# OthmanB/TAMCMC-C

Measured on AMD Instinct MI355X. Metric: MCMC samples/sec (whole node), 1e5 nu-bins x 100 params x 20 tempered chains, higher is better.
Workload: dtype f64

## Files before the change

### tamcmc-c_amd/csrc/dev_step_impl.h

```cpp

struct FusedArgs {
    int NS;
    int xsplit;
    double *cand_vars, *cand_params;
    double *cand_logPr;
    int *cand_rej;
    int *cand_stP, *cand_stR;
    tamcmc_multiplet *mults;
    int *pairs, *nh, *nn;
    double *noise;
    double *bg;
    int *slot;
    double *prop_logPr;
    int *prop_st;
    double *quick;
    double *part;
    double *psum;
    double *lz;
    double qmargin;
    unsigned long long *qcount;
};

constexpr int QN = 8;
constexpr int ST_L = 1, ST_BR = 2, ST_ENTRY = 4, ST_LZ = 8, ST_FIRST = 16, ST_COMMIT = 32;
// ... 117 lines not shown
        if (stm == TAMCMC_OK && !(lp == -INFINITY || isnan(lp))) {
            const double cur = settled ? a.logPost_cur[q * C + m] : d.o.logPost;
            Sstar = -((log(u) - lp + cur) * Tm) / (double)a.pl;
            if (isfinite(Sstar)) ok = 1;
        } else if (u > 0.0) ok = 2;
        w[0] = Sstar; w[1] = ok; w[2] = -(double)a.pl / Tm; w[3] = settled ? a.logL_cur[q * C + m] : d.o.logL;
        double lus = 0, k1 = 0, k2 = 0;
        if (is_swap_iter(a, it)) {
            double us;
            if (swap_first(a, it, &us) == m) {
                const double TB = a.Tcoefs[m + 1];
                lus = log(us); k1 = Tm / TB - 1.0; k2 = TB / Tm - 1.0;
            }
        }
        w[4] = lus; w[5] = k1; w[6] = k2; w[7] = (double)slot;
    }
    if (settled) return;
    const double *sv, *sp;
    if (d.src_acc) {
        const size_t gp = (size_t)((it - 1) % 3) * f.NS + d.src_ps;
        sv = f.cand_vars + gp * Nv;
        sp = f.cand_params + gp * Np;
    } else {
        sv = a.vars_cur + ((size_t)d.src_par * C + d.src) * Nv;
        sp = a.params_cur + ((size_t)d.src_par * C + d.src) * Np;
    }
    double *dv = a.vars_cur + ((size_t)q * C + m) * Nv, *dp = a.params_cur + ((size_t)q * C + m) * Np;
    double *rv = (a.samples && rec >= 0) ? a.samples + ((size_t)rec * C + m) * Nv : nullptr;
    for (int i = lane; i < Nv; i += 64) { const double v = sv[i]; dv[i] = v; if (rv) rv[i] = v; }
    for (int i = lane; i < Np; i += 64) dp[i] = sp[i];
    if (lane == 0) {
        a.logL_cur[q * C + m] = d.o.logL;
        a.logPr_cur[q * C + m] = d.o.logPr;
        a.logPost_cur[q * C + m] = d.o.logPost;
        f.slot[q * C + m] = slot;
        a.moved[m] = d.src_acc;
        a.Pmove[m] = d.r;
        if (m == 0 && d.src_acc) a.counters[1] += 1;
        a.counters[8 + m] += d.src_acc;
        if (m == 0) a.counters[0] = it;
        if (d.swap_first == m) {
            atomicAdd((unsigned long long *)&a.counters[2], 1ull);
            if (d.swapped) atomicAdd((unsigned long long *)&a.counters[3], 1ull);
        }
        if (a.stats && rec >= 0) {
            double *r = a.stats + ((size_t)rec * C + m) * 3;
            r[0] = d.o.logL; r[1] = d.o.logPr; r[2] = d.o.logPost;
        }
        if (tiles && d.swap_first < 0 && f.quick[((size_t)(q ^ 1) * C + m) * QN + 1] == 2.0) atomicAdd(f.qcount + 1, 1ull);
    }
}


template <bool PAIR>
__device__ __forceinline__ void quick_sums(const double *c0, int n, int lane, double &s0, double &a0, double &s1, double &a1) {
    for (int t0 = 0; t0 < n; t0 += 256) {
        double v[4], w[4];
#pragma unroll
        for (int k = 0; k < 4; k++) {
            const int t = t0 + k * 64 + lane;
            v[k] = t < n ? c0[t] : 0.0;
            if (PAIR) w[k] = t < n ? c0[n + t] : 0.0;
        }
#pragma unroll
        for (int k = 0; k < 4; k++) {
            s0 += v[k]; a0 += fabs(v[k]);
            if (PAIR) { s1 += w[k]; a1 += fabs(w[k]); }
        }
    }
#pragma unroll
    for (int off = 32; off >= 1; off >>= 1) {
        s0 += __shfl_xor(s0, off, 64); a0 += __shfl_xor(a0, off, 64);
        if (PAIR) { s1 += __shfl_xor(s1, off, 64); a1 += __shfl_xor(a1, off, 64); }
    }
}
__device__ __forceinline__ int quick_decide_core(const DevSamplerArgs *ga, const FusedArgs *gf, int m, int q, int pairA, Decided *out) {
    const ConstArgs &a = *(const ConstArgs *)uniform_ptr(ga);
    const ConstFused &f = *(const ConstFused *)uniform_ptr(gf);
    const int lane = threadIdx.x & 63, C = a.C;
    const int p = q ^ 1, n = a.ntiles;
    const bool in_pair = pairA >= 0 && (m == pairA || m == pairA + 1);
    const int j0 = in_pair ? pairA : m;
    const double *c0 = f.psum + ((size_t)p * C + j0) * n;
    const double *r0 = f.quick + ((size_t)p * C + j0) * QN;
    double rec, s0 = 0, a0 = 0, s1 = 0, a1 = 0;
    if (in_pair) {
        rec = lane < 2 * QN ? r0[lane] : 0.0;
        quick_sums<true>(c0, n, lane, s0, a0, s1, a1);
    } else {
        rec = lane < QN ? r0[lane] : 0.0;
        quick_sums<false>(c0, n, lane, s0, a0, s1, a1);
    }
    const double St0 = __shfl(rec, 0, 64), ok0 = __shfl(rec, 1, 64);
    const int ps0 = (int)__shfl(rec, 7, 64);
    const double mg = f.qmargin;
    int acc0 = 0;
    if (ok0 == 2.0) { s0 = 0; a0 = 0; }
    else if (ok0 > 0 && fabs(s0 - St0) > mg * (a0 + fabs(St0))) acc0 = s0 < St0 ? 1 : 0;
    else return -1;
    Decided d;
    d.swap_first = -1; d.swapped = 0; d.src_par = p; d.r = 0;
    d.o.acc = 0; d.o.r = 0; d.o.logL = 0; d.o.logPr = 0; d.o.logPost = 0;
    if (!in_pair) { d.slot = 2 * m + acc0; d.src = m; d.src_acc = acc0; d.src_ps = ps0; }
    else {
        const double St1 = __shfl(rec, QN, 64), ok1 = __shfl(rec, QN + 1, 64);
        const int ps1 = (int)__shfl(rec, QN + 7, 64);
        int acc1 = 0;
        if (ok1 == 2.0) { s1 = 0; a1 = 0; }
        else if (ok1 > 0 && fabs(s1 - St1) > mg * (a1 + fabs(St1))) acc1 = s1 < St1 ? 1 : 0;
        else return -1;
        const double c0 = __shfl(rec, 2, 64), c1 = __shfl(rec, QN + 2, 64);
        const double LA = acc0 ? c0 * s0 : __shfl(rec, 3, 64), LB = acc1 ? c1 * s1 : __shfl(rec, QN + 3, 64);
        const double lus = __shfl(rec, 4, 64), x = LA * __shfl(rec, 5, 64) + LB * __shfl(rec, 6, 64);
        if (!(fabs(x - lus) > mg * (fabs(c0) * a0 + fabs(c1) * a1 + fabs(LA) + fabs(LB)))) return -1;
        const int swapped = x > lus ? 1 : 0;
        const int A = pairA, B = pairA + 1;
        d.swap_first = A; d.swapped = swapped;
        if (swapped) {
            if (m == A) { d.slot = 2 * C + (A >= f.xsplit ? 4 : 0) + acc1; d.src = B; d.src_acc = acc1; d.src_ps = ps1; }
            else { d.slot = 2 * C + (B >= f.xsplit ? 4 : 0) + 2 + acc0; d.src = A; d.src_acc = acc0; d.src_ps = ps0; }
        } else {
            if (m == A) { d.slot = 2 * A + acc0; d.src = A; d.src_acc = acc0; d.src_ps = ps0; }
            else { d.slot = 2 * B + acc1; d.src = B; d.src_acc = acc1; d.src_ps = ps1; }
        }
    }
    if (out && lane == 0) *out = d;
    return d.slot;
}
__device__ __attribute__((noinline)) int quick_decide_leaf(const DevSamplerArgs *ga, const FusedArgs *gf, int m, int q, int pairA, Decided *out) {
    return quick_decide_core(ga, gf, m, q, pairA, out);
}

__device__ __forceinline__ int quick_decide(const DevSamplerArgs *ga, const FusedArgs *gf, int m, long it, int q, int settled, int pairA,
                                            Decided *out) {
    if (settled) return decide(ga, gf, m, it, q, 1, out);
    const int s = quick_decide_leaf(ga, gf, m, q, pairA, out);
    return s >= 0 ? s : decide(ga, gf, m, it, q, 0, out);
}

__device__ __attribute__((noinline)) int decide_counted(const DevSamplerArgs *ga, const FusedArgs *gf, int m, long it, int q, int tile) {
    if (tile == 0 && (threadIdx.x & 63) == 0) atomicAdd(((const ConstFused *)uniform_ptr(gf))->qcount, 1ull);
    return decide(ga, gf, m, it, q, 0, nullptr);
}

struct StepTiles {
    const DevSamplerArgs *ga;
    const FusedArgs *gf;
    long it;
    int q, first, settled, pairA;
    static constexpr bool coherent_partials = false;
    static constexpr bool early_loads = true;
    __device__ __forceinline__ tile::SlotWords head(const LoglikeArgs &a, int b, int tile) const {
        const int m = first + b;
        if (settled) return tile::slot_words(a, decide(ga, gf, m, it, q, 1, nullptr));
        const bool lone = a.per > 0 && !(pairA >= 0 && (m == pairA || m == pairA + 1));
        tile::SlotWords w0{}, w1{};
        if (lone) { w0 = tile::slot_words(a, 2 * m); w1 = tile::slot_words(a, 2 * m + 1); }
        int s = quick_decide_core(ga, gf, m, q, pairA, nullptr);
        if (s < 0) s = decide_counted(ga, gf, m, it, q, tile);
        if (lone && (s >> 1) == m) return (s & 1) ? w1 : w0;
        return tile::slot_words(a, s);
    }
    __device__ __forceinline__ void store_sums(int b, int tile, double s0, double s1) const {
        const ConstArgs &a = *(const ConstArgs *)uniform_ptr(ga);
        const ConstFused &f = *(const ConstFused *)uniform_ptr(gf);
        f.psum[((size_t)q * a.C + first + b) * a.ntiles + tile] = s0 + s1;
    }
    __device__ __forceinline__ void operator()(int, int, int) const {}
};

__device__ __attribute__((noinline)) void role_prior(const DevSamplerArgs *ga, const FusedArgs *gf, size_t gs, int h, const double *s_vars,
                                                     const double *s_params, const UnpackLds *Up) {
    const DevSamplerArgs &a = *ga;
    const FusedArgs &f = *gf;
    const UnpackLds U = *Up;
    const int Nv = a.Nv, Np = a.desc.Np, tid = threadIdx.x;
    if (h == 0) {
        for (int i = tid; i < Nv; i += 64) f.cand_vars[gs * Nv + i] = s_vars[i];
        for (int i = tid; i < Np; i += 64) f.cand_params[gs * Np + i] = s_params[i];
    }
    int rej = 0;
#ifdef TAMCMC_PROBE
    long ps_[4] = {0, 0, 0, 0};
    const double fh = wave_log_prior_part(a.desc, s_params, U, TB - 128, h, &rej, ps_);
    if (tid == 0 && (int)(gs % f.NS) == 2) { long *w = a.counters + 8 + a.C + 16 * h + 4; w[0] += ps_[1] - ps_[0]; w[1] += ps_[2] - ps_[1]; }
#else
    const double fh = wave_log_prior_part(a.desc, s_params, U, TB - 128, h, &rej);
#endif
    if (tid == 0) {
        f.cand_logPr[2 * gs + h] = fh;
        f.cand_stP[2 * gs + h] = *U.status;
        if (h == 0) f.cand_rej[gs] = rej;
    }
}
__device__ __forceinline__ TablePtrs candidate_tables(const DevSamplerArgs &a, const FusedArgs &f, int q_dst) {
    TablePtrs T;
    T.mults = f.mults + (size_t)q_dst * f.NS * a.desc.per; T.pairs = f.pairs + (size_t)q_dst * 2 * f.NS; T.nh = f.nh + (size_t)q_dst * f.NS;
    T.nn = f.nn + (size_t)q_dst * f.NS; T.noise = f.noise + (size_t)q_dst * f.NS * a.desc.stride;
    T.bg = nullptr; T.ntiles = a.ntiles; T.tile_bins = a.tile_bins;
    return T;
}
__device__ __attribute__((noinline)) void role_rows(const DevSamplerArgs *ga, const FusedArgs *gf, int q_dst, int slot, size_t gs,
                                                    const double *s_params, const UnpackLds *Up) {
    const DevSamplerArgs &a = *ga;
    const FusedArgs &f = *gf;
    const UnpackLds U = *Up;
    if (threadIdx.x == 0) mt::shared_scalars_base(a.desc.model_id, s_params, a.desc.plength, *U.S);
    __syncthreads();
    const TablePtrs T = candidate_tables(a, f, q_dst);
#ifdef TAMCMC_PROBE
    __shared__ long ps_[8];
    wg_unpack(a.desc, s_params, U, slot, T, true, false, false, true, ps_);
    __syncthreads();
    if (threadIdx.x == 0 && (int)(gs % f.NS) == 2) {
        long *w = a.counters + 8 + a.C + 8 + 4; w[0] += ps_[1] - ps_[0]; w[1] += ps_[2] - ps_[1];
        long *v = a.counters + 8 + a.C + 32; v[0] += ps_[5] - ps_[4]; v[1] += ps_[6] - ps_[5]; v[2] += ps_[7] - ps_[6]; v[3] += 1;
    }
#else
    wg_unpack(a.desc, s_params, U, slot, T, true, false, false, true);
#endif
    if (threadIdx.x == 0) f.cand_stR[gs] = *U.status;
}
__device__ __attribute__((noinline)) void role_background(const DevSamplerArgs *ga, const FusedArgs *gf, int q_dst, int slot, int role,
                                                          const double *s_params, const UnpackLds *Up) {
    const DevSamplerArgs &a = *ga;
    const FusedArgs &f = *gf;
    const UnpackLds U = *Up;
    if (!f.bg) return;
    if (threadIdx.x == 0) mt::shared_scalars_base(a.desc.model_id, s_params, a.desc.plength, *U.S);
    __syncthreads();
    TablePtrs T = candidate_tables(a, f, q_dst);
    T.bg = f.bg + (size_t)q_dst * f.NS * a.ntiles * bg::NH;
    const int quarter = (a.ntiles + 3) / 4, k = role - 3;
    wg_bg_tiles(a.desc, s_params, U.S, slot, T, 0, 64, k * quarter, (k + 1) * quarter);
}

__device__ __attribute__((noinline)) void lz_normals(const DevSamplerArgs *ga, long itn, int m, double *s_z) {
    normals_into(*ga, m, itn, s_z);
}
__device__ __attribute__((noinline)) void lz_rows(const DevSamplerArgs *ga, const FusedArgs *gf, int q_dst, int m, const double *s_z) {
    Lz_rows_wave(*ga, m, s_z, gf->lz + ((size_t)q_dst * ga->C + m) * ga->Nv);
}
__device__ __forceinline__ void lz_block(const DevSamplerArgs *ga, const FusedArgs *gf, long itn, int q_dst, int m, unsigned char *lds) {
    double *s_z = (double *)lds;
    lz_normals(ga, itn, m, s_z);
    __syncthreads();
    lz_rows(ga, gf, q_dst, m, s_z);
}

__device__ void candidate_role(const DevSamplerArgs &a, const FusedArgs &f, const DevSamplerArgs *ga, const FusedArgs *gf, long itn, int q_src,
                               int q_dst, int slot, int role, bool entry, int settled, int pairA, unsigned char *lds, Decided *dec) {
    if (role > 6) return;
    const int C = a.C, Nv = a.Nv, Np = a.desc.Np, tid = threadIdx.x;
    const int e_dst = (int)(itn % 3);
    int m, src, on_prop;
    if (slot < 2 * C) { m = slot >> 1; src = m; on_prop = slot & 1; }
    else {
        if (entry || !is_swap_iter(a, itn - 1)) return;
        const int A = swap_first(a, itn - 1, nullptr), e = slot - 2 * C;
        m = (e < 2) ? A : A + 1;
        src = (e < 2) ? A + 1 : A;
        on_prop = e & 1;
        slot += (m >= f.xsplit) ? 4 : 0;
    }
    if (entry && on_prop) return;
    if (entry && role == 0 && tid == 0) f.slot[q_src * C + m] = 2 * m;
#ifdef TAMCMC_PROBE
    long pt[6];
    pt[0] = (long)wall_clock64();
#define RSTAMP(k) pt[k] = (long)wall_clock64()
#else
#define RSTAMP(k)
#endif
    double *s_params = (double *)lds;
    double *s_vars = s_params + Np;
    double *s_z = s_vars + Nv;
    const UnpackLds U = carve_unpack_lds((unsigned char *)(s_z + Nv + 1));
    __shared__ UnpackLds s_U;
    if (tid == 0) s_U = U;
    const double *bv, *bp;
    if (entry) {
        bv = a.vars_cur + ((size_t)q_src * C + src) * Nv;
        bp = a.params_cur + ((size_t)q_src * C + src) * Np;
    } else {
        const int ps = quick_decide(ga, gf, src, itn - 1, q_src, settled, pairA, dec);
        __syncthreads();
        const Decided d = *dec;
        if (on_prop) {
            const size_t gp = (size_t)((itn - 1) % 3) * f.NS + ps;
            bv = f.cand_vars + gp * Nv;
            bp = f.cand_params + gp * Np;
        } else if (d.src_acc) {
            const size_t gp = (size_t)((itn - 2) % 3) * f.NS + d.src_ps;
            bv = f.cand_vars + gp * Nv;
            bp = f.cand_params + gp * Np;
        } else {
            bv = a.vars_cur + ((size_t)d.src_par * C + d.src) * Nv;
            bp = a.params_cur + ((size_t)d.src_par * C + d.src) * Np;
        }
    }
    RSTAMP(1);
    const double *lz = f.lz + ((size_t)q_dst * C + m) * Nv;
    constexpr int PW = (int)(sizeof(mt::PolyTab) / sizeof(double));
    if (Nv <= 128 && Np <= 128 && PW <= 256) {
        double r_v[2], r_z[2], r_p[2], r_t[4];
        int r_i[2];
#pragma unroll
        for (int e = 0; e < 2; e++) {
            const int i = tid + 64 * e;
            r_v[e] = i < Nv ? bv[i] : 0.0; r_z[e] = i < Nv ? lz[i] : 0.0; r_i[e] = i < Nv ? a.index_to_relax[i] : 0;
            r_p[e] = i < Np ? bp[i] : 0.0;
        }
// ... 108 lines not shown
```

### tamcmc-c_amd/csrc/loglike_tile.h

```cpp
#pragma once
#include <hip/hip_runtime.h>
#include <stdint.h>

#include "kernels.h"
#include "bg_series.h"

namespace tamcmc {
namespace tile {

constexpr int CHUNK = 64;

constexpr int F_FULL = 1;
constexpr int F_SAFE = 2;
constexpr int F_ASYM = 4;
constexpr int F_FAR = 8;

constexpr int M_STRICT = 0, M_FAST_DIRECT = 2, M_FAST = 1;

constexpr int NC = 16;
constexpr double RHO_MAX2 = 1.0 / 36.0;
constexpr double RHO_MAX2_ASYM = 1.0 / 64.0;
constexpr int NH = bg::NH;
constexpr int ROW = NC + 2;

struct __attribute__((aligned(16))) LdsMult {
    int i0, i1, l, flags;
    double g;
    double asym;
    double c2sq;
    double fcx;
    double2 nh[7];
};

__device__ __forceinline__ double rcp_nr1(double d) {
    double r = __builtin_amdgcn_rcp(d);
    return fma(fma(-d, r, 1.0), r, r);
}
__device__ __forceinline__ double rcp_nr2(double d) {
    double r = __builtin_amdgcn_rcp(d);
    r = fma(fma(-d, r, 1.0), r, r);
    return fma(fma(-d, r, 1.0), r, r);
}

template <int NV, int WGS = 256>
__device__ __forceinline__ void block_reduce(double (&v)[NV], double *s_red, double *out) {
    const int lane = threadIdx.x & 63, wave = threadIdx.x >> 6;
#pragma unroll
    for (int i = 0; i < NV; i++) {
#pragma unroll
        for (int off = 32; off >= 1; off >>= 1) v[i] = v[i] + __shfl_down(v[i], off, 64);
    }
    if (lane == 0) {
#pragma unroll
        for (int i = 0; i < NV; i++) s_red[wave * NV + i] = v[i];
    }
    __syncthreads();
    if (threadIdx.x == 0) {
#pragma unroll
        for (int i = 0; i < NV; i++) {
            double s = s_red[i];
            for (int w = 1; w < WGS / 64; w++) s = s + s_red[w * NV + i];
            out[i] = s;
        }
    }
}

template <int NM, int K, bool FULL>
__device__ __forceinline__ void strict_mult(const LdsMult &M, const double (&xv)[K], const int (&bin)[K], double (&acc)[K]) {
    double nu[NM], hv[NM];
#pragma unroll
    for (int m = 0; m < NM; m++) {
        const double2 p = M.nh[m];
        nu[m] = p.x;
        hv[m] = p.y;
    }
    const double g2 = M.g;
    const int i0 = M.i0, i1 = M.i1;
    if (!(M.flags & F_ASYM)) {
#pragma unroll
        for (int k = 0; k < K; k++) {
            if (FULL || (bin[k] >= i0 && bin[k] < i1)) {
                double res = 0.0;
#pragma unroll
                for (int m = 0; m < NM; m++) {
                    const double d = xv[k] - nu[m];
                    double p = d * d;
                    p = 4.0 * p / g2;
                    const double inv = 1.0 / (1.0 + p);
                    res = res + hv[m] * inv;
                }
                acc[k] = acc[k] + res;
            }
        }
    } else {
        const double asym = M.asym, fc = M.fcx, c2sq = M.c2sq;
#pragma unroll
        for (int k = 0; k < K; k++) {
            if (FULL || (bin[k] >= i0 && bin[k] < i1)) {
                const double t = 1.0 + asym * (xv[k] / fc - 1.0);
                const double asy = t * t + c2sq;
                double res = 0.0;
#pragma unroll
                for (int m = 0; m < NM; m++) {
                    const double d = xv[k] - nu[m];
                    double p = d * d;
                    p = 4.0 * p / g2;
                    const double inv = 1.0 / (1.0 + p);
                    res = res + hv[m] * (asy * inv);
                }
                acc[k] = acc[k] + res;
            }
        }
    }
}

template <int NM, int K, bool FULL>
__device__ __forceinline__ void fast_mult(const LdsMult &M, const double (&xv)[K], const int (&bin)[K], double (&acc)[K], double xc) {
    double nA[NM], hv[NM];
#pragma unroll
    for (int m = 0; m < NM; m++) {
        const double2 p = M.nh[m];
        nA[m] = -p.x;
        hv[m] = p.y;
    }
    const double g = M.g;
    const int i0 = M.i0, i1 = M.i1;
    const int flags = M.flags;
    if (flags & F_SAFE) {
        const bool has_asym = flags & F_ASYM;
        const double afc = M.fcx, c2sq = M.c2sq, one_m_asym = 1.0 - M.asym;
#pragma unroll
        for (int k = 0; k < K; k++) {
            if (FULL || (bin[k] >= i0 && bin[k] < i1)) {
                const double xx = xv[k];
                const double dx = xx - xc;
                double t = fma(dx, g, nA[0]);
                double D = fma(t, t, 1.0);
                double N = hv[0];
#pragma unroll
                for (int m = 1; m < NM; m++) {
                    t = fma(dx, g, nA[m]);
                    const double q = fma(t, t, 1.0);
                    N = fma(N, q, hv[m] * D);
                    D = D * q;
                }
                double res = N * rcp_nr1(D);
                if (has_asym) {
                    const double ta = fma(afc, xx, one_m_asym);
                    res = res * fma(ta, ta, c2sq);
                }
                acc[k] = acc[k] + res;
            }
            if (K > 4 && (k & 3) == 3) __builtin_amdgcn_sched_barrier(0);
        }
    } else {
#pragma unroll
        for (int k = 0; k < K; k++) {
            if (FULL || (bin[k] >= i0 && bin[k] < i1)) {
                const double xx = xv[k];
                const double dx = xx - xc;
                double res = 0.0;
#pragma unroll
                for (int m = 0; m < NM; m++) {
                    const double t = fma(dx, g, nA[m]);
                    res = res + hv[m] / fma(t, t, 1.0);
                }
                if (flags & F_ASYM) {
                    const double ta = fma(M.fcx, xx, 1.0 - M.asym);
                    res = res * fma(ta, ta, M.c2sq);
                }
                acc[k] = acc[k] + res;
            }
        }
    }
}

template <bool FAST, int NM, int K>
__device__ __forceinline__ void mult_dispatch(const LdsMult &M, const double (&xv)[K], const int (&bin)[K], double (&acc)[K], double xc) {
    if (M.flags & F_FULL) {
        if (FAST) fast_mult<NM, K, true>(M, xv, bin, acc, xc);
        else strict_mult<NM, K, true>(M, xv, bin, acc);
    } else {
        if (FAST) fast_mult<NM, K, false>(M, xv, bin, acc, xc);
        else strict_mult<NM, K, false>(M, xv, bin, acc);
    }
}


template <int MODE, int WGS>
struct __attribute__((aligned(16))) TileLds {
    static constexpr bool FARFIELD = (MODE == M_FAST);
    static constexpr int LDS_BYTES = FARFIELD ? (WGS * ROW * 8 > CHUNK * (int)sizeof(LdsMult) ? WGS * ROW * 8 : CHUNK * (int)sizeof(LdsMult))
                                              : CHUNK * (int)sizeof(LdsMult);
    unsigned char buf[LDS_BYTES];
    double coef[NC];
    double part[WGS / 16][NC];
    double red[2 * (WGS / 64)];
    double lt[TAMCMC_MAX_HARVEY];
    double lto[TAMCMC_MAX_HARVEY];
    int n, nfar, anyfar;
    unsigned short slot[CHUNK * 7];
};

template <int MODE, int WGS, int K, bool WRITE_MODEL, bool DELTA, class Tail>
__device__ __forceinline__ void tile_compute(const LoglikeArgs &a, const int tile, const int b, const int sb, TileLds<MODE, WGS> &S, const int mbeg,
                                             const int mend, const int nh, const int nn, const Tail &tail, const double *xpre) {
    constexpr bool FAST = (MODE != M_STRICT);
    constexpr bool COH = Tail::coherent_partials;
    static_assert(!DELTA || (FAST && !WRITE_MODEL), "DELTA launches are FAST-mode, logL-only");
    constexpr bool FARFIELD = (MODE == M_FAST);
    LdsMult *s_m = (LdsMult *)S.buf;
    double *s_rows = (double *)S.buf;
    int &s_n = S.n, &s_nfar = S.nfar, &s_anyfar = S.anyfar;
    unsigned short *s_slot = S.slot;
    double *s_coef = S.coef;
    double(*s_part)[NC] = S.part;
    double *s_red = S.red;
    double *s_lt = S.lt, *s_lto = S.lto;
    const int tid = threadIdx.x;
#ifdef TAMCMC_PROBE
#define KSTAMP(k) do { if (a.dbg && b == 0 && tile == a.ntiles / 2 && tid == 0) a.dbg[k] = (long)wall_clock64(); } while (0)
#define PROBE_SKIP(bit) (a.probe & (bit))
    const long wg_t0 = (a.dbg && a.dbg[7] == 77) ? (long)wall_clock64() : 0;
#else
#define KSTAMP(k) do { } while (0)
#define PROBE_SKIP(bit) false
#endif
    KSTAMP(0);
    constexpr int TILE = WGS * K;
    const int t0 = tile * TILE;
    const int t1 = min(t0 + TILE, a.Nx);
    if (DELTA) {
        if (a.d_done && a.d_done[(size_t)b * a.ntiles + tile]) return;
        const int lo = a.d_range[2 * b], hi = a.d_range[2 * b + 1];
        if (t1 <= lo || t0 >= hi) {
            if (tid == 0) {
                double *p = a.partials + ((size_t)b * a.ntiles + tile) * 2;
                p[0] = 0.0;
                p[1] = 0.0;
            }
            return;
        }
    }

    tamcmc_multiplet g;
    const bool fullnew = DELTA && (a.d_flags[b] & 2);
    const bool dsub = DELTA && !fullnew;
    const bool bg_prebuilt = FARFIELD && a.bg_poly && (!DELTA || fullnew);
    double bg_pre = 0.0;
    if (bg_prebuilt && tid < NH) bg_pre = a.bg_poly[((size_t)(DELTA ? a.d_row[b] : sb) * a.ntiles + tile) * NH + tid];
    double xv[K], yv[K], acc[K];
    int bin[K];
#pragma unroll
    for (int k = 0; k < K; k++) {
        bin[k] = t0 + k * WGS + tid;
        const int bi = min(bin[k], a.Nx - 1);
        xv[k] = xpre ? xpre[k] : a.x[bi];
        acc[k] = 0.0;
    }

    const double *nz = a.noise + (size_t)sb * a.noise_stride;
    const bool bg = !DELTA || fullnew || (a.d_flags[b] & 1);
    const double *nzo = DELTA ? a.d_noise_old + (size_t)b * a.noise_stride : nz;
    const double h = 0.5 * (double)TILE * a.step;
    const double xc = a.x0 + ((double)t0 + 0.5 * (double)TILE - 0.5) * a.step;
    const bool harvey_poly = FARFIELD && bg && bg::series_valid(xc, h);
    if (FAST && bg && !harvey_poly) {
        if (tid < nh) {
            s_lt[tid] = log(1e-3 * nz[3 * tid + 1]);
            if (dsub) s_lto[tid] = log(1e-3 * nzo[3 * tid + 1]);
        }
    }
    if (FARFIELD) {
        if (tid < NC) s_coef[tid] = 0.0;
        if (tid == 0) s_anyfar = harvey_poly ? 1 : 0;
        __syncthreads();
        if (harvey_poly && !bg_prebuilt) {
            const int hl = (WGS > 64) ? tid - 64 : tid;
            double f[NH];
#pragma unroll
            for (int k = 0; k < NH; k++) f[k] = 0.0;
            const bool lane_new = (hl >= 0 && hl < nh), lane_old = dsub && (hl >= 32 && hl < 32 + nh);
            if (lane_new || lane_old) {
                const double *nq = lane_new ? nz : nzo;
                const int ht = lane_new ? hl : hl - 32;
                bg::harvey_term_series(lane_new ? nq[3 * ht] : -nq[3 * ht], nq[3 * ht + 1], nq[3 * ht + 2], xc, h, f);
            }
            if (hl >= 0 && hl < 64) {
#pragma unroll
                for (int k = 0; k < NH; k++) {
                    double v = f[k];
                    double tot = 0.0;
                    for (int t = 0; t < nh; t++) tot = tot + __shfl(v, t, 64);
                    if (dsub)
                        for (int t = 0; t < nh; t++) tot = tot + __shfl(v, 32 + t, 64);
                    const double wn = dsub ? (nz[nn - 1] - nzo[nn - 1]) : nz[nn - 1];
                    if (hl == 0) s_coef[k] = tot + (k == 0 ? wn : 0.0);
                }
            }
        }
    }

    bool bg_in_regs = harvey_poly && bg_prebuilt;
    bool any_near = false;
    KSTAMP(1);
    for (int c0 = mbeg; c0 < mend; c0 += CHUNK) {
        __syncthreads();
        if (tid < 64) {
            const int idx = c0 + tid;
            g = a.mults[a.per > 0 ? min(idx, mbeg + a.per - 1) : min(idx, mend - 1)];
            const int i0 = g.i0, i1 = g.i1;
            const bool ov = (idx < mend) && (i0 < t1) && (i1 > t0) && !PROBE_SKIP(16);
            const int l = g.l;
            const int nm = 2 * l + 1;
            const bool full = (i0 <= t0 && i1 >= t1);
            bool far = false;
            if (FARFIELD && ov && full) {
                const double ig = 2.0 * rcp_nr2(g.gamma);
                const double beta2 = (ig * h) * (ig * h);
                const double r2 = (g.asym != 0.0) ? RHO_MAX2_ASYM : RHO_MAX2;
                far = true;
#pragma unroll
                for (int m = 0; m < 7; m++) {
                    const double A = ig * (g.nu[m] - xc);
                    if (m < nm && !(beta2 <= r2 * fma(A, A, 1.0))) far = false;
                }
            }
            const unsigned long long mask = __ballot(ov);
            const unsigned long long fmask = FARFIELD ? __ballot(far) : 0ull;
            const unsigned long long lt = (1ull << tid) - 1ull;
            const int n_near = __popcll(mask & ~fmask);
            const int pos = far ? n_near + __popcll(fmask & lt) : __popcll(mask & ~fmask & lt);
            if (ov) {
                LdsMult &d = s_m[pos];
                int flags = 0;
                if (full) flags |= F_FULL;
                if (g.asym != 0.0) flags |= F_ASYM;
                const double ifc = FAST ? rcp_nr2(g.fc) : 0.0;
                const double c2 = FAST ? 0.5 * g.gamma * g.asym * ifc : 0.5 * g.gamma * g.asym / g.fc;
                d.c2sq = c2 * c2;
                d.asym = g.asym;
                double Am[7];
                if (FAST) {
                    const double ig = 2.0 * rcp_nr2(g.gamma);
                    d.g = ig;
                    d.fcx = g.asym * ifc;
#pragma unroll
                    for (int m = 0; m < 7; m++) Am[m] = ig * (g.nu[m] - xc);
                    if (far) flags |= F_FAR;
                    else {
                        const double bh = ig * h;
                        bool safe = true;
#pragma unroll
                        for (int m = 0; m < 7; m++) {
                            const double dm = fabs(Am[m]) + bh;
                            if (m < nm && !(fma(dm, dm, 1.0) < 1e38)) safe = false;
                        }
                        if (safe) flags |= F_SAFE;
                    }
                } else {
                    d.g = g.gamma * g.gamma;
                    d.fcx = g.fc;
                }
                d.i0 = i0; d.i1 = i1; d.l = l; d.flags = flags;
#pragma unroll
                for (int m = 0; m < 7; m++) d.nh[m] = make_double2(FAST ? Am[m] : g.nu[m], g.hv[m]);
            }
            if (FARFIELD) {
                const int lv = ov ? g.l : 0;
                const unsigned long long f0 = __ballot(far && lv == 0), f1 = __ballot(far && lv == 1), f2 = __ballot(far && lv == 2),
                                         f3 = __ballot(far && lv >= 3);
                if (far) {
                    const int off = __popcll(f0 & lt) + 3 * __popcll(f1 & lt) + 5 * __popcll(f2 & lt) + 7 * __popcll(f3 & lt);
                    const int nmf = 2 * (lv > 3 ? 3 : lv) + 1;
                    for (int m = 0; m < nmf; m++) s_slot[off + m] = (unsigned short)((pos << 3) | m);
                }
                if (tid == 0) {
                    s_nfar = __popcll(f0) + 3 * __popcll(f1) + 5 * __popcll(f2) + 7 * __popcll(f3);
                    if (f0 | f1 | f2 | f3) s_anyfar = 1;
                }
            }
            if (tid == 0) s_n = n_near;
        }
        __syncthreads();
        KSTAMP(2);
        const int n = PROBE_SKIP(1) ? 0 : s_n;
        any_near = any_near || (s_n > 0);
        for (int q = 0; q < n; q++) {
            const LdsMult &M = s_m[q];
            switch (M.l) {
            case 0: mult_dispatch<FAST, 1, K>(M, xv, bin, acc, xc); break;
            case 1: mult_dispatch<FAST, 3, K>(M, xv, bin, acc, xc); break;
            case 2: mult_dispatch<FAST, 5, K>(M, xv, bin, acc, xc); break;
            default: mult_dispatch<FAST, 7, K>(M, xv, bin, acc, xc); break;
            }
        }
        KSTAMP(3);
        if (FARFIELD && s_nfar > 0 && !PROBE_SKIP(2)) {
            double fcoef[NC];
#pragma unroll
            for (int k = 0; k < NC; k++) fcoef[k] = 0.0;
            const int nslots = s_nfar;
            for (int slot = tid; slot < nslots; slot += WGS) {
                const int e = s_slot[slot];
                const LdsMult &M = s_m[e >> 3];
                {
                    const double2 nhm = M.nh[e & 7];
                    const double beta = M.g * h;
                    const double A = nhm.x;
                    const double inv = rcp_nr2(fma(A, A, 1.0));
                    const double two_req = 2.0 * beta * A * inv, q2 = beta * beta * inv;
                    double cm = nhm.y * inv;
                    double cc = cm * two_req;
                    if (!(M.flags & F_ASYM)) {
                        fcoef[0] = fcoef[0] + cm;
                        fcoef[1] = fcoef[1] + cc;
                        const int nt = (q2 > 1.39e-2) ? 16 : (q2 > 6.8e-3) ? 14 : (q2 > 2.5e-3) ? 12 : (q2 > 5.6e-4) ? 10 : (q2 > 4.6e-5) ? 8 : 6;
#pragma unroll
                        for (int k = 2; k < NC; k++) {
                            if ((k & 1) == 0 && k >= 6 && !__any(k < nt)) break;
                            const double cn = fma(two_req, cc, -q2 * cm);
                            fcoef[k] = fcoef[k] + cn;
                            cm = cc;
                            cc = cn;
                        }
                    } else {
                        const double p0 = fma(M.fcx, xc, 1.0 - M.asym), p1 = M.fcx * h;
                        const double A0 = fma(p0, p0, M.c2sq), A1 = 2.0 * p0 * p1, A2 = p1 * p1;
                        double c2 = 0.0, c1 = 0.0, c0k = cm;
                        double nxt = cc;
#pragma unroll
                        for (int k = 0; k < NC; k++) {
                            fcoef[k] = fcoef[k] + fma(A0, c0k, fma(A1, c1, A2 * c2));
                            const double cn = (k == 0) ? nxt : fma(two_req, c0k, -q2 * c1);
                            c2 = c1;
                            c1 = c0k;
                            c0k = cn;
                        }
                    }
                }
            }
            __syncthreads();
#pragma unroll
            for (int k = 0; k < NC; k += 2) *(double2 *)&s_rows[tid * ROW + k] = make_double2(fcoef[k], fcoef[k + 1]);
            __syncthreads();
            {
                const int k = tid & 15, part = tid >> 4;
                double sum = 0.0;
#pragma unroll
                for (int r = 0; r < 16; r++) sum = sum + s_rows[(part * 16 + r) * ROW + k];
                s_part[part][k] = sum;
            }
            __syncthreads();
            if (tid < NC) {
                double sum = (bg_in_regs && tid < NH) ? bg_pre : s_coef[tid];
#pragma unroll
                for (int p = 0; p < WGS / 16; p++) sum = sum + s_part[p][tid];
                s_coef[tid] = sum;
            }
            bg_in_regs = false;
        }
    }
    if (bg_in_regs && tid < NH) s_coef[tid] = bg_pre;
    KSTAMP(4);
#pragma unroll
    for (int k = 0; k < K; k++) yv[k] = DELTA ? 0.0 : a.y[min(bin[k], a.Nx - 1)];
    if (FAST) __syncthreads();
    if constexpr (DELTA && FARFIELD && WGS == 64) {
        if (a.fd_mom && (!bg || harvey_poly) && !fullnew && !any_near) {
            const double *mm = a.fd_mom + ((size_t)a.d_row[b] * a.ntiles + tile) * FD_MOM;
            const double w1 = (tid < NC) ? mm[tid] : 0.0, w2 = (tid < 2 * NC - 1) ? mm[NC + tid] : 0.0, rmax = mm[FD_MOM - 1];
            const double ck = (tid < NC) ? s_coef[tid] : 0.0;
            double ab = fabs(ck);
#pragma unroll
            for (int off = 32; off >= 1; off >>= 1) ab = ab + __shfl_xor(ab, off, 64);
            if (ab * rmax <= 1e-5) {
                double cv = 0.0;
                if (tid < 2 * NC - 1) {
                    const int j0 = tid < NC ? 0 : tid - (NC - 1), j1 = tid < NC ? tid : NC - 1;
                    for (int j = j0; j <= j1; j++) cv = fma(s_coef[j], s_coef[tid - j], cv);
                }
                double tot = fma(ck, w1, cv * w2);
#pragma unroll
                for (int off = 32; off >= 1; off >>= 1) tot = tot + __shfl_xor(tot, off, 64);
                if (tid == 0) {
                    double *p = a.partials + ((size_t)b * a.ntiles + tile) * 2;
                    p[0] = tot;
                    p[1] = 0.0;
                }
                return;
            }
        }
    }
    if (FARFIELD) {
        if (s_anyfar && !PROBE_SKIP(4)) {
            const double inv_h = 1.0 / h;
#pragma unroll
            for (int k = 0; k < K; k++) {
                const double sx = (xv[k] - xc) * inv_h;
                double P = s_coef[NC - 1];
#pragma unroll
                for (int q = NC - 2; q >= 0; q--) P = fma(P, sx, s_coef[q]);
                acc[k] = acc[k] + P;
            }
        }
    }

    KSTAMP(5);
    double s[2] = {0.0, 0.0};
    const double white = nz[nn - 1];
    double prod = 1.0, ynum = 0.0;
    double Mk[K];
#pragma unroll
    for (int k = 0; k < K; k++) {
        double Mv = acc[k];
        const int bi = min(bin[k], a.Nx - 1);
        const bool valid = bin[k] < a.Nx;
        if (!FAST) {
            for (int hh = 0; hh < nh; hh++) {
                const double tau = nz[3 * hh + 1];
                if (tau != 0.0) {
                    double t = pow((1e-3 * tau) * xv[k], nz[3 * hh + 2]);
                    t = nz[3 * hh] * (1.0 / (t + 1.0));
                    Mv = Mv + t;
                }
            }
            Mv = Mv + white;
            if (valid) {
                s[0] = s[0] + yv[k] * (1.0 / Mv);
                s[1] = s[1] + log(Mv);
            }
        } else {
            if (bg && !harvey_poly) {
                const double lx = a.logx[bi];
                for (int hh = 0; hh < nh; hh++) {
                    const double tau = nz[3 * hh + 1];
                    if (tau != 0.0) {
                        const double t = exp(nz[3 * hh + 2] * (s_lt[hh] + lx));
                        Mv = fma(nz[3 * hh], rcp_nr2(t + 1.0), Mv);
                    }
                    if (dsub) {
                        const double tauo = nzo[3 * hh + 1];
                        if (tauo != 0.0) {
                            const double t = exp(nzo[3 * hh + 2] * (s_lto[hh] + lx));
                            Mv = fma(-nzo[3 * hh], rcp_nr2(t + 1.0), Mv);
                        }
                    }
                }
                Mv = Mv + (dsub ? (white - nzo[nn - 1]) : white);
            }
            if (DELTA) {
                const size_t o = (size_t)a.d_row[b] * a.Nx + (size_t)min(bin[k], a.Nx - 1);
                const double r0 = a.model0[o], yr = a.model0[a.fd_plane + o];
                const double u = (fullnew ? Mv - a.model0[2 * a.fd_plane + o] : Mv) * r0;
                double f;
                if (!__any(valid && !(fabs(u) <= 0.01))) {
                    double pz = fma(u, 0.2 - yr, yr - 0.25);
                    pz = fma(u, pz, (1.0 / 3.0) - yr);
                    pz = fma(u, pz, yr - 0.5);
                    pz = fma(u, pz, 1.0 - yr);
                    f = u * pz;
                } else f = fma(-yr * u, rcp_nr2(1.0 + u), log1p(u));
                if (valid) s[0] = s[0] + f;
            } else if (valid) {
                if (PROBE_SKIP(8)) s[0] = s[0] + yv[k] * Mv;
                else {
                    ynum = fma(ynum, Mv, yv[k] * prod);
                    prod = prod * Mv;
                }
            }
        }
        Mk[k] = Mv;
        if (WRITE_MODEL) {
            if (valid) {
                if (a.fd_rows) {
                    const double r0 = FAST ? rcp_nr2(Mv) : 1.0 / Mv;
                    a.fd_rows[(size_t)b * a.Nx + bin[k]] = r0;
                    a.fd_rows[a.fd_plane + (size_t)b * a.Nx + bin[k]] = yv[k] * r0;
                    a.fd_rows[2 * a.fd_plane + (size_t)b * a.Nx + bin[k]] = Mv;
                } else a.model[(size_t)b * a.Nx + bin[k]] = Mv;
            }
        }
    }
    if (FAST && !DELTA) {
        if (prod > 1e-280 && prod < 1e280) {
            s[1] = log(prod);
            s[0] = s[0] + ynum * rcp_nr2(prod);
        } else {
#pragma unroll
            for (int k = 0; k < K; k++)
                if (bin[k] < a.Nx) {
                    s[1] = s[1] + log(Mk[k]);
                    s[0] = fma(yv[k], rcp_nr2(Mk[k]), s[0]);
                }
        }
    }
    __syncthreads();
    double out[2];
    block_reduce<2, WGS>(s, s_red, out);
    if (tid == 0) {
        double *p = a.partials + ((size_t)b * a.ntiles + tile) * 2;
        if (COH) {
            typedef double __attribute__((address_space(1))) *gdp_t;
            __hip_atomic_store((gdp_t)p, out[0], __ATOMIC_RELAXED, __HIP_MEMORY_SCOPE_AGENT);
            __hip_atomic_store((gdp_t)p + 1, out[1], __ATOMIC_RELAXED, __HIP_MEMORY_SCOPE_AGENT);
        } else {
            p[0] = out[0];
            p[1] = out[1];
        }
        tail.store_sums(b, tile, out[0], out[1]);
    }
    KSTAMP(6);
#ifdef TAMCMC_PROBE
    if (a.dbg && a.dbg[7] == 77 && tid == 0) {
        long *w = a.dbg + 8 + 2 * ((size_t)b * a.ntiles + tile);
        w[0] = wg_t0;
        w[1] = (long)wall_clock64();
    }
#endif
#undef KSTAMP
#undef PROBE_SKIP
}

struct SlotWords { int sb, nn, nh, mbeg, mend; };
__device__ __forceinline__ SlotWords slot_words(const LoglikeArgs &a, int sb) {
    SlotWords w;
    w.sb = sb; w.nn = a.nnoise[sb]; w.nh = a.nharvey[sb];
    w.mend = a.offsets[2 * sb + 1];
    w.mbeg = a.per > 0 ? (a.slot0 + sb) * a.per : a.offsets[2 * sb];
    return w;
}

struct NoTail {
    static constexpr bool coherent_partials = false;
    static constexpr bool early_loads = false;
    __device__ __forceinline__ int slot(const LoglikeArgs &, int b, int ) const { return b; }
    __device__ __forceinline__ void store_sums(int , int , double, double) const {}
    __device__ __forceinline__ void operator()(int , int , int ) const {}
};

template <int MODE, int WGS, int K, bool WRITE_MODEL, bool DELTA, class Tail>
__device__ __forceinline__ void loglike_tile(const LoglikeArgs &a, const int id, TileLds<MODE, WGS> &S, const Tail &tail) {
    const int xcd = id & 7;
    int j = id >> 3, b, tile;
    if (a.prio_b < 0) {
        b = j % a.B;
        tile = (j / a.B) * 8 + xcd;
    } else {
        const int lead = ((a.ntiles + 7) >> 3) * 2;
        if (j < lead) {
            b = a.prio_b + (j & 1);
            tile = (j >> 1) * 8 + xcd;
        } else {
            j -= lead;
            const int rest = a.B - 2, r = j % rest;
            b = r + (r >= a.prio_b ? 2 : 0);
            tile = (j / rest) * 8 + xcd;
        }
    }
    if (tile >= a.ntiles) return;
    tile += a.tile_rot;
    if (tile >= a.ntiles) tile -= a.ntiles;
    SlotWords w;
    double xpre[Tail::early_loads ? K : 1];
    if constexpr (Tail::early_loads) {
#pragma unroll
        for (int k = 0; k < K; k++) xpre[k] = a.x[min(tile * (WGS * K) + k * WGS + (int)threadIdx.x, a.Nx - 1)];
        w = tail.head(a, b, tile);
    } else w = slot_words(a, tail.slot(a, b, tile));
    if (w.nn > 0)
        tile_compute<MODE, WGS, K, WRITE_MODEL, DELTA, Tail>(a, tile, b, w.sb, S, w.mbeg, w.mend, w.nh, w.nn, tail, Tail::early_loads ? xpre : nullptr);
    tail(b, tile, w.sb);
}

}
}
```

Before: 49020.

## Prefetch y early, drop per-bin index arrays, add full-tile fast path

Replaces the per-element bin index array with one base index plus compile-time offsets, which frees registers and removes the min() clamps on full tiles. The observation y values are now prefetched alongside x before the slot decision, so their load latency overlaps the decide logic. Model writes and the delta-mode reads take a specialised full-tile path with plain strided addressing. The slot index is also made wave-uniform with readfirstlane so it lives in scalar registers. In exchange, early prefetching keeps more values live across the decide call and duplicates the terms loop into two instantiations.

Result: no change. 48870 (-0.3%).

```diff
diff --git a/tamcmc-c_amd/csrc/dev_step_impl.h b/tamcmc-c_amd/csrc/dev_step_impl.h
--- a/tamcmc-c_amd/csrc/dev_step_impl.h
+++ b/tamcmc-c_amd/csrc/dev_step_impl.h
@@ -293,12 +293,13 @@
     static constexpr bool early_loads = true;
     __device__ __forceinline__ tile::SlotWords head(const LoglikeArgs &a, int b, int tile) const {
         const int m = first + b;
-        if (settled) return tile::slot_words(a, decide(ga, gf, m, it, q, 1, nullptr));
+        if (settled) return tile::slot_words(a, __builtin_amdgcn_readfirstlane(decide(ga, gf, m, it, q, 1, nullptr)));
         const bool lone = a.per > 0 && !(pairA >= 0 && (m == pairA || m == pairA + 1));
         tile::SlotWords w0{}, w1{};
         if (lone) { w0 = tile::slot_words(a, 2 * m); w1 = tile::slot_words(a, 2 * m + 1); }
         int s = quick_decide_core(ga, gf, m, q, pairA, nullptr);
         if (s < 0) s = decide_counted(ga, gf, m, it, q, tile);
+        s = __builtin_amdgcn_readfirstlane(s);
         if (lone && (s >> 1) == m) return (s & 1) ? w1 : w0;
         return tile::slot_words(a, s);
     }
diff --git a/tamcmc-c_amd/csrc/loglike_tile.h b/tamcmc-c_amd/csrc/loglike_tile.h
--- a/tamcmc-c_amd/csrc/loglike_tile.h
+++ b/tamcmc-c_amd/csrc/loglike_tile.h
@@ -1,6 +1,7 @@
 #pragma once
 #include <hip/hip_runtime.h>
 #include <stdint.h>
+#include <type_traits>
 
 #include "kernels.h"
 #include "bg_series.h"
@@ -65,8 +66,8 @@
     }
 }
 
-template <int NM, int K, bool FULL>
-__device__ __forceinline__ void strict_mult(const LdsMult &M, const double (&xv)[K], const int (&bin)[K], double (&acc)[K]) {
+template <int NM, int K, int WGS, bool FULL>
+__device__ __forceinline__ void strict_mult(const LdsMult &M, const double (&xv)[K], const int tb, double (&acc)[K]) {
     double nu[NM], hv[NM];
 #pragma unroll
     for (int m = 0; m < NM; m++) {
@@ -79,7 +80,7 @@
     if (!(M.flags & F_ASYM)) {
 #pragma unroll
         for (int k = 0; k < K; k++) {
-            if (FULL || (bin[k] >= i0 && bin[k] < i1)) {
+            if (FULL || (tb >= i0 - k * WGS && tb < i1 - k * WGS)) {
                 double res = 0.0;
 #pragma unroll
                 for (int m = 0; m < NM; m++) {
@@ -96,7 +97,7 @@
         const double asym = M.asym, fc = M.fcx, c2sq = M.c2sq;
 #pragma unroll
         for (int k = 0; k < K; k++) {
-            if (FULL || (bin[k] >= i0 && bin[k] < i1)) {
+            if (FULL || (tb >= i0 - k * WGS && tb < i1 - k * WGS)) {
                 const double t = 1.0 + asym * (xv[k] / fc - 1.0);
                 const double asy = t * t + c2sq;
                 double res = 0.0;
@@ -114,8 +115,8 @@
     }
 }
 
-template <int NM, int K, bool FULL>
-__device__ __forceinline__ void fast_mult(const LdsMult &M, const double (&xv)[K], const int (&bin)[K], double (&acc)[K], double xc) {
+template <int NM, int K, int WGS, bool FULL>
+__device__ __forceinline__ void fast_mult(const LdsMult &M, const double (&xv)[K], const int tb, double (&acc)[K], double xc) {
     double nA[NM], hv[NM];
 #pragma unroll
     for (int m = 0; m < NM; m++) {
@@ -131,7 +132,7 @@
         const double afc = M.fcx, c2sq = M.c2sq, one_m_asym = 1.0 - M.asym;
 #pragma unroll
         for (int k = 0; k < K; k++) {
-            if (FULL || (bin[k] >= i0 && bin[k] < i1)) {
+            if (FULL || (tb >= i0 - k * WGS && tb < i1 - k * WGS)) {
                 const double xx = xv[k];
                 const double dx = xx - xc;
                 double t = fma(dx, g, nA[0]);
@@ -156,7 +157,7 @@
     } else {
 #pragma unroll
         for (int k = 0; k < K; k++) {
-            if (FULL || (bin[k] >= i0 && bin[k] < i1)) {
+            if (FULL || (tb >= i0 - k * WGS && tb < i1 - k * WGS)) {
                 const double xx = xv[k];
                 const double dx = xx - xc;
                 double res = 0.0;
@@ -175,14 +176,27 @@
     }
 }
 
-template <bool FAST, int NM, int K>
-__device__ __forceinline__ void mult_dispatch(const LdsMult &M, const double (&xv)[K], const int (&bin)[K], double (&acc)[K], double xc) {
+template <bool FAST, int NM, int K, int WGS>
+__device__ __forceinline__ void mult_dispatch(const LdsMult &M, const double (&xv)[K], const int tb, double (&acc)[K], double xc) {
     if (M.flags & F_FULL) {
-        if (FAST) fast_mult<NM, K, true>(M, xv, bin, acc, xc);
-        else strict_mult<NM, K, true>(M, xv, bin, acc);
+        if (FAST) fast_mult<NM, K, WGS, true>(M, xv, tb, acc, xc);
+        else strict_mult<NM, K, WGS, true>(M, xv, tb, acc);
     } else {
-        if (FAST) fast_mult<NM, K, false>(M, xv, bin, acc, xc);
-        else strict_mult<NM, K, false>(M, xv, bin, acc);
+        if (FAST) fast_mult<NM, K, WGS, false>(M, xv, tb, acc, xc);
+        else strict_mult<NM, K, WGS, false>(M, xv, tb, acc);
+    }
+}
+
+template <int WGS, int K>
+__device__ __forceinline__ void load_bins(const double *p, const int tb, const int Nx, const bool full_tile, double (&v)[K]) {
+    if (full_tile) {
+        const double *q = p + tb;
+#pragma unroll
+        for (int k = 0; k < K; k++) v[k] = q[k * WGS];
+        asm volatile("");
+    } else {
+#pragma unroll
+        for (int k = 0; k < K; k++) v[k] = p[min(tb + k * WGS, Nx - 1)];
     }
 }
 
@@ -204,7 +218,7 @@
 
 template <int MODE, int WGS, int K, bool WRITE_MODEL, bool DELTA, class Tail>
 __device__ __forceinline__ void tile_compute(const LoglikeArgs &a, const int tile, const int b, const int sb, TileLds<MODE, WGS> &S, const int mbeg,
-                                             const int mend, const int nh, const int nn, const Tail &tail, const double *xpre) {
+                                             const int mend, const int nh, const int nn, const Tail &tail, const double *xpre, const double *ypre) {
     constexpr bool FAST = (MODE != M_STRICT);
     constexpr bool COH = Tail::coherent_partials;
     static_assert(!DELTA || (FAST && !WRITE_MODEL), "DELTA launches are FAST-mode, logL-only");
@@ -250,14 +264,14 @@
     double bg_pre = 0.0;
     if (bg_prebuilt && tid < NH) bg_pre = a.bg_poly[((size_t)(DELTA ? a.d_row[b] : sb) * a.ntiles + tile) * NH + tid];
     double xv[K], yv[K], acc[K];
-    int bin[K];
-#pragma unroll
-    for (int k = 0; k < K; k++) {
-        bin[k] = t0 + k * WGS + tid;
-        const int bi = min(bin[k], a.Nx - 1);
-        xv[k] = xpre ? xpre[k] : a.x[bi];
-        acc[k] = 0.0;
-    }
+    const int tb = t0 + tid;
+    const bool full_tile = (t1 - t0 == TILE);
+    if (xpre) {
+#pragma unroll
+        for (int k = 0; k < K; k++) xv[k] = xpre[k];
+    } else load_bins<WGS, K>(a.x, tb, a.Nx, full_tile, xv);
+#pragma unroll
+    for (int k = 0; k < K; k++) acc[k] = 0.0;
 
     const double *nz = a.noise + (size_t)sb * a.noise_stride;
     const bool bg = !DELTA || fullnew || (a.d_flags[b] & 1);
@@ -389,10 +403,10 @@
         for (int q = 0; q < n; q++) {
             const LdsMult &M = s_m[q];
             switch (M.l) {
-            case 0: mult_dispatch<FAST, 1, K>(M, xv, bin, acc, xc); break;
-            case 1: mult_dispatch<FAST, 3, K>(M, xv, bin, acc, xc); break;
-            case 2: mult_dispatch<FAST, 5, K>(M, xv, bin, acc, xc); break;
-            default: mult_dispatch<FAST, 7, K>(M, xv, bin, acc, xc); break;
+            case 0: mult_dispatch<FAST, 1, K, WGS>(M, xv, tb, acc, xc); break;
+            case 1: mult_dispatch<FAST, 3, K, WGS>(M, xv, tb, acc, xc); break;
+            case 2: mult_dispatch<FAST, 5, K, WGS>(M, xv, tb, acc, xc); break;
+            default: mult_dispatch<FAST, 7, K, WGS>(M, xv, tb, acc, xc); break;
             }
         }
         KSTAMP(3);
@@ -463,8 +477,10 @@
     }
     if (bg_in_regs && tid < NH) s_coef[tid] = bg_pre;
     KSTAMP(4);
-#pragma unroll
-    for (int k = 0; k < K; k++) yv[k] = DELTA ? 0.0 : a.y[min(bin[k], a.Nx - 1)];
+    if (DELTA || ypre) {
+#pragma unroll
+        for (int k = 0; k < K; k++) yv[k] = DELTA ? 0.0 : ypre[k];
+    } else load_bins<WGS, K>(a.y, tb, a.Nx, full_tile, yv);
     if (FAST) __syncthreads();
     if constexpr (DELTA && FARFIELD && WGS == 64) {
         if (a.fd_mom && (!bg || harvey_poly) && !fullnew && !any_near) {
@@ -514,8 +530,6 @@
 #pragma unroll
     for (int k = 0; k < K; k++) {
         double Mv = acc[k];
-        const int bi = min(bin[k], a.Nx - 1);
-        const bool valid = bin[k] < a.Nx;
         if (!FAST) {
             for (int hh = 0; hh < nh; hh++) {
                 const double tau = nz[3 * hh + 1];
@@ -526,33 +540,44 @@
                 }
             }
             Mv = Mv + white;
-            if (valid) {
-                s[0] = s[0] + yv[k] * (1.0 / Mv);
-                s[1] = s[1] + log(Mv);
-            }
-        } else {
-            if (bg && !harvey_poly) {
-                const double lx = a.logx[bi];
-                for (int hh = 0; hh < nh; hh++) {
-                    const double tau = nz[3 * hh + 1];
-                    if (tau != 0.0) {
-                        const double t = exp(nz[3 * hh + 2] * (s_lt[hh] + lx));
-                        Mv = fma(nz[3 * hh], rcp_nr2(t + 1.0), Mv);
+        } else if (bg && !harvey_poly) {
+            const double lx = a.logx[min(tb + k * WGS, a.Nx - 1)];
+            for (int hh = 0; hh < nh; hh++) {
+                const double tau = nz[3 * hh + 1];
+                if (tau != 0.0) {
+                    const double t = exp(nz[3 * hh + 2] * (s_lt[hh] + lx));
+                    Mv = fma(nz[3 * hh], rcp_nr2(t + 1.0), Mv);
+                }
+                if (dsub) {
+                    const double tauo = nzo[3 * hh + 1];
+                    if (tauo != 0.0) {
+                        const double t = exp(nzo[3 * hh + 2] * (s_lto[hh] + lx));
+                        Mv = fma(-nzo[3 * hh], rcp_nr2(t + 1.0), Mv);
                     }
-                    if (dsub) {
-                        const double tauo = nzo[3 * hh + 1];
-                        if (tauo != 0.0) {
-                            const double t = exp(nzo[3 * hh + 2] * (s_lto[hh] + lx));
-                            Mv = fma(-nzo[3 * hh], rcp_nr2(t + 1.0), Mv);
-                        }
-                    }
-                }
-                Mv = Mv + (dsub ? (white - nzo[nn - 1]) : white);
-            }
-            if (DELTA) {
-                const size_t o = (size_t)a.d_row[b] * a.Nx + (size_t)min(bin[k], a.Nx - 1);
-                const double r0 = a.model0[o], yr = a.model0[a.fd_plane + o];
-                const double u = (fullnew ? Mv - a.model0[2 * a.fd_plane + o] : Mv) * r0;
+                }
+            }
+            Mv = Mv + (dsub ? (white - nzo[nn - 1]) : white);
+        }
+        Mk[k] = Mv;
+    }
+    auto terms = [&](auto FT) {
+        constexpr bool FULLT = decltype(FT)::value;
+        const size_t row0 = DELTA ? (size_t)a.d_row[b] * a.Nx : 0;
+        const double *m0 = DELTA ? a.model0 + row0 + tb : nullptr;
+        double *wq = WRITE_MODEL ? (a.fd_rows ? a.fd_rows : a.model) + (size_t)b * a.Nx + tb : nullptr;
+#pragma unroll
+        for (int k = 0; k < K; k++) {
+            const double Mv = Mk[k];
+            const bool valid = FULLT || tb < a.Nx - k * WGS;
+            if (!FAST) {
+                if (valid) {
+                    s[0] = s[0] + yv[k] * (1.0 / Mv);
+                    s[1] = s[1] + log(Mv);
+                }
+            } else if (DELTA) {
+                const double *mo = FULLT ? m0 + k * WGS : a.model0 + row0 + min(tb + k * WGS, a.Nx - 1);
+                const double r0 = mo[0], yr = mo[a.fd_plane];
+                const double u = (fullnew ? Mv - mo[2 * a.fd_plane] : Mv) * r0;
                 double f;
                 if (!__any(valid && !(fabs(u) <= 0.01))) {
                     double pz = fma(u, 0.2 - yr, yr - 0.25);
@@ -569,19 +594,20 @@
                     prod = prod * Mv;
                 }
             }
-        }
-        Mk[k] = Mv;
-        if (WRITE_MODEL) {
-            if (valid) {
-                if (a.fd_rows) {
-                    const double r0 = FAST ? rcp_nr2(Mv) : 1.0 / Mv;
-                    a.fd_rows[(size_t)b * a.Nx + bin[k]] = r0;
-                    a.fd_rows[a.fd_plane + (size_t)b * a.Nx + bin[k]] = yv[k] * r0;
-                    a.fd_rows[2 * a.fd_plane + (size_t)b * a.Nx + bin[k]] = Mv;
-                } else a.model[(size_t)b * a.Nx + bin[k]] = Mv;
-            }
-        }
-    }
+            if (WRITE_MODEL) {
+                if (valid) {
+                    if (a.fd_rows) {
+                        const double r0 = FAST ? rcp_nr2(Mv) : 1.0 / Mv;
+                        wq[k * WGS] = r0;
+                        wq[a.fd_plane + k * WGS] = yv[k] * r0;
+                        wq[2 * a.fd_plane + k * WGS] = Mv;
+                    } else wq[k * WGS] = Mv;
+                }
+            }
+        }
+    };
+    if (full_tile) terms(std::true_type{});
+    else terms(std::false_type{});
     if (FAST && !DELTA) {
         if (prod > 1e-280 && prod < 1e280) {
             s[1] = log(prod);
@@ -589,7 +615,7 @@
         } else {
 #pragma unroll
             for (int k = 0; k < K; k++)
-                if (bin[k] < a.Nx) {
+                if (full_tile || tb < a.Nx - k * WGS) {
                     s[1] = s[1] + log(Mk[k]);
                     s[0] = fma(yv[k], rcp_nr2(Mk[k]), s[0]);
                 }
@@ -662,14 +688,17 @@
     tile += a.tile_rot;
     if (tile >= a.ntiles) tile -= a.ntiles;
     SlotWords w;
-    double xpre[Tail::early_loads ? K : 1];
+    double xpre[Tail::early_loads ? K : 1], ypre[Tail::early_loads && !DELTA ? K : 1];
     if constexpr (Tail::early_loads) {
-#pragma unroll
-        for (int k = 0; k < K; k++) xpre[k] = a.x[min(tile * (WGS * K) + k * WGS + (int)threadIdx.x, a.Nx - 1)];
+        const int t0 = tile * (WGS * K);
+        const bool full_tile = (a.Nx - t0 >= WGS * K);
+        load_bins<WGS, K>(a.x, t0 + (int)threadIdx.x, a.Nx, full_tile, xpre);
+        if constexpr (!DELTA) load_bins<WGS, K>(a.y, t0 + (int)threadIdx.x, a.Nx, full_tile, ypre);
         w = tail.head(a, b, tile);
     } else w = slot_words(a, tail.slot(a, b, tile));
     if (w.nn > 0)
-        tile_compute<MODE, WGS, K, WRITE_MODEL, DELTA, Tail>(a, tile, b, w.sb, S, w.mbeg, w.mend, w.nh, w.nn, tail, Tail::early_loads ? xpre : nullptr);
+        tile_compute<MODE, WGS, K, WRITE_MODEL, DELTA, Tail>(a, tile, b, w.sb, S, w.mbeg, w.mend, w.nh, w.nn, tail, Tail::early_loads ? xpre : nullptr,
+                                                             Tail::early_loads && !DELTA ? ypre : nullptr);
     tail(b, tile, w.sb);
 }
 
```
